# lblQubic/distributed_processor

Measured on AMD Instinct MI355X. Metric: emulated core-shots/s (config 2: 8-core Ramsey, 100 delays, 1e6 shots/GPU), higher is better.
Workload: dtype u32; 1 GPU; config2_ramsey_8core_100pt; shots_per_gpu=1000000, lane_order=shot-major, parallelism=shots sharded, 1 GPU(s)

## Files before the change

distributed_processor_amd/csrc/capi.cpp:

```cpp

#include <hip/hip_runtime.h>

#include <algorithm>
#include <cmath>
#include <cstdarg>
#include <cstdio>
#include <cstring>
#include <initializer_list>
#include <string>
#include <vector>

#include "kernels.h"
#include "launch_plan.h"
#include "lds_grants.h"
#include "program_image.h"

using namespace dpemu;

namespace dpemu {
static LdsGrants g_lds_grants;

hipError_t opt_in_dynamic_lds(const void *fn, size_t bytes)
{
    if (bytes <= LdsGrants::DEFAULT_LIMIT) return hipSuccess;
// ... 48 lines not shown
    uint32_t n_cu = 256;
    std::string err;
    uint4 *d_uops = nullptr;
    uint4 *d_uops_t = nullptr;
    uint4 *d_macro = nullptr;
    uint32_t *d_moff = nullptr;
    uint32_t *d_mchunk = nullptr, *d_mcoff = nullptr;
    uint32_t *d_offsets = nullptr, *d_ninstr = nullptr, *d_table = nullptr;
    ProgramFacts facts;
    uint32_t *d_ro_fq = nullptr;
    uint4 *d_ro_hdr = nullptr;
    uint32_t *d_thr = nullptr;
    uint64_t *d_lut = nullptr;
    std::vector<uint32_t> thr_cache;
    std::vector<uint64_t> lut_cache;
    int16_t *d_sin = nullptr;
    DevTable ch;
    DevTable dds_index;
    DevTable pairs;
    DevTable lines, fl_index;
    DevTable res;
    DevTable iqcols;
    uint32_t iq_wgs_per_cu = 0;
    DevTable trace_tab;
    uint32_t trace_wgs_per_cu = 0;
    DevTable qsim_tab;
    std::string last_kernel;
    bool timing = false;
    std::vector<std::pair<hipEvent_t, hipEvent_t>> ev_used, ev_free;
    DevTable hist_rep;
    bool hist_rep_dirty = true;
    hipEvent_t ord_ev = nullptr;
    hipStream_t ord_stream = nullptr;
    bool ord_valid = false;
};

static int fail(dpemu_ctx *ctx, int code, const char *fmt, ...)
{
    char buf[512];
    va_list ap;
    va_start(ap, fmt);
    vsnprintf(buf, sizeof buf, fmt, ap);
    va_end(ap);
    if (ctx) ctx->err = buf;
    return code;
}

#define HIPCHK(ctx, call)                                                                  \
    do {                                                                                   \
        hipError_t e_ = (call);                                                            \
        if (e_ != hipSuccess)                                                              \
            return fail(ctx, DPEMU_E_DEVICE, "%s: %s", #call, hipGetErrorString(e_));      \
    } while (0)

struct NamedPtr { const void *p; const char *name; };
static int check_ptrs(dpemu_ctx *ctx, const char *what, std::initializer_list<NamedPtr> ptrs)
{
    for (const NamedPtr &a : ptrs)
        if (a.name && !a.p) return fail(ctx, DPEMU_E_INVALID, "%s: %s is NULL", what, a.name);
    return DPEMU_OK;
}

static hipError_t order_begin(dpemu_ctx *ctx, hipStream_t s)
{
    if (ctx->ord_valid && s != ctx->ord_stream) return hipStreamWaitEvent(s, ctx->ord_ev, 0);
    return hipSuccess;
}

static hipError_t order_end(dpemu_ctx *ctx, hipStream_t s)
{
    const hipError_t e = hipEventRecord(ctx->ord_ev, s);
    ctx->ord_stream = s;
    ctx->ord_valid = e == hipSuccess;
    return e;
}

template <class Launch> static hipError_t timed(dpemu_ctx *ctx, hipStream_t stream, Launch launch)
{
    if (!ctx->timing) return launch();
    std::pair<hipEvent_t, hipEvent_t> e;
    if (!ctx->ev_free.empty()) {
        e = ctx->ev_free.back();
        ctx->ev_free.pop_back();
    } else {
        hipError_t r = hipEventCreate(&e.first);
        if (r != hipSuccess) return r;
        r = hipEventCreate(&e.second);
        if (r != hipSuccess) { (void)hipEventDestroy(e.first); return r; }
    }
    ctx->ev_used.push_back(e);
    hipError_t r = hipEventRecord(e.first, stream);
    if (r == hipSuccess) r = launch();
    if (r == hipSuccess) r = hipEventRecord(e.second, stream);
    return r;
}

template <class P> static void set_readout(P &p, const dpemu_config *cfg)
{
    p.seed = cfg->seed;
    p.meas_elem = cfg->meas_elem; p.ro_cpw = cfg->ro_cpw; p.ro_delay = cfg->ro_delay;
    p.ro_theta0 = cfg->ro_theta[0]; p.ro_theta1 = cfg->ro_theta[1];
    p.ro_gain0 = cfg->ro_gain[0]; p.ro_gain1 = cfg->ro_gain[1];
    p.ro_sigma = cfg->ro_sigma; p.ro_thr = cfg->ro_thr;
}

template <class T> static hipError_t to_device(T *&d, const uint32_t *src, uint64_t n)
{
// ... 31 lines not shown
    return DPEMU_OK;
}

int dpemu_create(int device, dpemu_ctx **out)
{
    if (!out) return DPEMU_E_INVALID;
    *out = nullptr;
    int n = 0;
    if (hipGetDeviceCount(&n) != hipSuccess || device < 0 || device >= n) return DPEMU_E_DEVICE;
    if (hipSetDevice(device) != hipSuccess) return DPEMU_E_DEVICE;
    dpemu_ctx *ctx = new dpemu_ctx();
    ctx->device = device;
    int cus = 0;
    if (hipDeviceGetAttribute(&cus, hipDeviceAttributeMultiprocessorCount, device) == hipSuccess && cus > 0)
        ctx->n_cu = (uint32_t)cus;
    std::vector<int16_t> lut(4096);
    dpemu_dds_sin_lut(lut.data());
    if (hipMalloc(&ctx->d_thr, 2 * DPEMU_MAX_CORES * sizeof(uint32_t)) != hipSuccess ||
        hipMalloc(&ctx->d_lut, 256 * sizeof(uint64_t)) != hipSuccess ||
        hipMalloc(&ctx->d_sin, 4096 * sizeof(int16_t)) != hipSuccess ||
        hipMemcpy(ctx->d_sin, lut.data(), 4096 * sizeof(int16_t), hipMemcpyHostToDevice) != hipSuccess ||
        hipEventCreateWithFlags(&ctx->ord_ev, hipEventDisableTiming) != hipSuccess) {
        dpemu_destroy(ctx);
        return DPEMU_E_NOMEM;
    }
    *out = ctx;
    return DPEMU_OK;
}

int dpemu_destroy(dpemu_ctx *ctx)
{
    if (!ctx) return DPEMU_E_INVALID;
    (void)hipSetDevice(ctx->device);
    if (ctx->ord_valid) (void)hipEventSynchronize(ctx->ord_ev);
    free_programs(ctx);
    (void)hipFree(ctx->d_thr); (void)hipFree(ctx->d_lut); (void)hipFree(ctx->d_sin);
    for (DevTable *t : {&ctx->ch, &ctx->dds_index, &ctx->pairs, &ctx->lines, &ctx->fl_index, &ctx->res, &ctx->iqcols,
                        &ctx->trace_tab, &ctx->qsim_tab, &ctx->hist_rep})
        t->release();
    for (auto *v : {&ctx->ev_used, &ctx->ev_free})
        for (auto &e : *v) { (void)hipEventDestroy(e.first); (void)hipEventDestroy(e.second); }
    if (ctx->ord_ev) (void)hipEventDestroy(ctx->ord_ev);
    delete ctx;
    return DPEMU_OK;
}

const char *dpemu_last_error(dpemu_ctx *ctx) { return ctx ? ctx->err.c_str() : "null context"; }

const char *dpemu_last_kernel(dpemu_ctx *ctx) { return ctx ? ctx->last_kernel.c_str() : ""; }

int dpemu_set_kernel_timing(dpemu_ctx *ctx, int enable)
{
    if (!ctx) return DPEMU_E_INVALID;
    ctx->timing = enable != 0;
    return DPEMU_OK;
}

int dpemu_kernel_times(dpemu_ctx *ctx, float *ms, int max_n, int *n_out)
{
    if (!ctx || (max_n > 0 && !ms)) return DPEMU_E_INVALID;
    HIPCHK(ctx, hipSetDevice(ctx->device));
    int n = 0;
    for (auto &e : ctx->ev_used) {
        HIPCHK(ctx, hipEventSynchronize(e.second));
        if (n < max_n) HIPCHK(ctx, hipEventElapsedTime(&ms[n], e.first, e.second));
        n++;
    }
    ctx->ev_free.insert(ctx->ev_free.end(), ctx->ev_used.begin(), ctx->ev_used.end());
    ctx->ev_used.clear();
    if (n_out) *n_out = n < max_n ? n : max_n;
    return DPEMU_OK;
}

int dpemu_load_programs(dpemu_ctx *ctx, const uint32_t *words, uint64_t n_cmds, const uint32_t *offsets,
                        const uint32_t *n_instr, uint32_t n_programs, const uint32_t *prog_table,
                        uint32_t n_groups, uint32_t cores_per_shot)
{
    if (!ctx) return DPEMU_E_INVALID;
    if ((!words && n_cmds) || !offsets || !n_instr || !prog_table || n_programs == 0 || n_groups == 0)
        return fail(ctx, DPEMU_E_INVALID, "load_programs: null array or empty program set");
    const uint32_t C = cores_per_shot;
    if (C == 0 || C > DPEMU_MAX_CORES || (C & (C - 1)))
        return fail(ctx, DPEMU_E_INVALID, "cores_per_shot %u is not a power of two in [1, 64]", C);
    if ((uint64_t)n_groups * C > 0xFFFFFFFFull) return fail(ctx, DPEMU_E_INVALID, "n_groups * C exceeds 2^32");
    for (uint32_t i = 0; i < n_programs; i++) {
        if (n_instr[i] > 65536u)
            return fail(ctx, DPEMU_E_INVALID, "program %u: %u commands exceed the 2^16-deep cmd_mem", i, n_instr[i]);
        if ((uint64_t)offsets[i] + n_instr[i] > n_cmds)
            return fail(ctx, DPEMU_E_INVALID, "program %u: offset %u + %u commands run past the %llu commands",
                        i, offsets[i], n_instr[i], (unsigned long long)n_cmds);
    }
    for (uint64_t i = 0; i < (uint64_t)n_groups * C; i++)
        if (prog_table[i] >= n_programs)
            return fail(ctx, DPEMU_E_INVALID, "prog_table[%llu] = %u >= n_programs", (unsigned long long)i, prog_table[i]);
    const ProgramImage im = build_program_image(words, offsets, n_instr, n_programs, prog_table, n_groups, C);
    if (!im.err.empty()) return fail(ctx, DPEMU_E_INVALID, "%s", im.err.c_str());
    HIPCHK(ctx, hipSetDevice(ctx->device));
    if (ctx->ord_valid) HIPCHK(ctx, hipEventSynchronize(ctx->ord_ev));
    free_programs(ctx);
    HIPCHK(ctx, to_device(ctx->d_uops, im.uops.data(), im.uops.size()));
    HIPCHK(ctx, to_device(ctx->d_uops_t, im.uops_t.data(), im.uops_t.size()));
    HIPCHK(ctx, to_device(ctx->d_macro, im.macro.data(), im.macro.size()));
    HIPCHK(ctx, to_device(ctx->d_moff, im.moff.data(), im.moff.size()));
    HIPCHK(ctx, to_device(ctx->d_mchunk, im.mchunk.data(), im.mchunk.size()));
    HIPCHK(ctx, to_device(ctx->d_mcoff, im.mcoff.data(), im.mcoff.size()));
    HIPCHK(ctx, to_device(ctx->d_offsets, im.goff.data(), n_programs));
    HIPCHK(ctx, to_device(ctx->d_ninstr, n_instr, n_programs));
    HIPCHK(ctx, to_device(ctx->d_table, prog_table, (uint64_t)n_groups * C));
    ctx->facts = im.facts;
    return DPEMU_OK;
}

int dpemu_load_readout_freqs(dpemu_ctx *ctx, const uint32_t *words, uint64_t n_words, const uint32_t *drv_off,
                             const uint32_t *drv_len, const uint32_t *lo_off, const uint32_t *lo_len)
{
    if (!ctx) return DPEMU_E_INVALID;
    if (!ctx->facts.n_programs) return fail(ctx, DPEMU_E_NOPROG, "load_readout_freqs before load_programs");
    if ((!words && n_words) || !drv_off || !drv_len || !lo_off || !lo_len)
        return fail(ctx, DPEMU_E_INVALID, "load_readout_freqs: null array");
    std::vector<uint32_t> hdr(4ull * ctx->facts.n_programs);
    for (uint32_t i = 0; i < ctx->facts.n_programs; i++) {
        if ((uint64_t)drv_off[i] + drv_len[i] > n_words || (uint64_t)lo_off[i] + lo_len[i] > n_words)
            return fail(ctx, DPEMU_E_INVALID, "load_readout_freqs: program %u's table runs past the %llu words", i,
                        (unsigned long long)n_words);
        hdr[4 * i] = drv_off[i]; hdr[4 * i + 1] = drv_len[i]; hdr[4 * i + 2] = lo_off[i]; hdr[4 * i + 3] = lo_len[i];
    }
    HIPCHK(ctx, hipSetDevice(ctx->device));
    if (ctx->ord_valid) HIPCHK(ctx, hipEventSynchronize(ctx->ord_ev));
    (void)hipFree(ctx->d_ro_fq);
    (void)hipFree(ctx->d_ro_hdr);
    ctx->d_ro_fq = nullptr;
    ctx->d_ro_hdr = nullptr;
    HIPCHK(ctx, hipMalloc(&ctx->d_ro_fq, std::max<uint64_t>(n_words, 1) * 4));
    if (n_words) HIPCHK(ctx, hipMemcpy(ctx->d_ro_fq, words, n_words * 4, hipMemcpyHostToDevice));
    HIPCHK(ctx, hipMalloc(&ctx->d_ro_hdr, hdr.size() * 4));
    HIPCHK(ctx, hipMemcpy(ctx->d_ro_hdr, hdr.data(), hdr.size() * 4, hipMemcpyHostToDevice));
    return DPEMU_OK;
}

static int validate(dpemu_ctx *ctx, const dpemu_config *cfg, uint64_t n_shots, bool want_hist)
{
    if (!cfg) return fail(ctx, DPEMU_E_INVALID, "null config");
    if (!ctx->facts.n_programs) return fail(ctx, DPEMU_E_NOPROG, "run before load_programs");
    if (cfg->cores_per_shot != ctx->facts.C)
        return fail(ctx, DPEMU_E_INVALID, "cores_per_shot %u != loaded %u", cfg->cores_per_shot, ctx->facts.C);
    if (cfg->n_groups != ctx->facts.n_groups)
        return fail(ctx, DPEMU_E_INVALID, "n_groups %u != loaded %u", cfg->n_groups, ctx->facts.n_groups);
    if (cfg->shots_per_group == 0) return fail(ctx, DPEMU_E_INVALID, "shots_per_group == 0");
    if (cfg->n_groups > 0x80000000u) return fail(ctx, DPEMU_E_INVALID, "n_groups > 2^31");
    if (cfg->max_cycles == 0 || cfg->max_cycles > 0x7FFFFFC0u)
        return fail(ctx, DPEMU_E_INVALID, "max_cycles must be in (0, 2^31 - 64]");
    if (cfg->meas_latency < 1 || cfg->meas_latency > (1u << 20) || cfg->sync_latency < 1 ||
        cfg->sync_latency > (1u << 20))
        return fail(ctx, DPEMU_E_INVALID, "meas_latency / sync_latency must be in [1, 2^20]");
    if (cfg->meas_model > DPEMU_MEAS_DEMOD)
        return fail(ctx, DPEMU_E_INVALID, "meas_model must be DPEMU_MEAS_STATE, _READOUT or _DEMOD");
    if (cfg->meas_model == DPEMU_MEAS_DEMOD) {
        if (cfg->ro_drv_elem > 3 || cfg->ro_drv_elem == cfg->meas_elem)
            return fail(ctx, DPEMU_E_INVALID, "ro_drv_elem %u must be an element 0..3 other than meas_elem",
                        cfg->ro_drv_elem);
        if (cfg->ro_cpw < 1 || cfg->ro_cpw > DPEMU_RO_CPW_MAX)
// ... 70 lines not shown
    p.n_shots = (uint32_t)n_shots;
    p.shot_major = cfg->lane_order == DPEMU_LANES_SHOT_MAJOR;
    p.C = C;
    p.log2C = 0;
    while ((1u << p.log2C) < C) p.log2C++;
    p.n_groups = cfg->n_groups; p.shots_per_group = cfg->shots_per_group;
    p.grp_g0 = (uint32_t)((shot_begin / cfg->shots_per_group) % cfg->n_groups);
    p.grp_r0 = (uint32_t)(shot_begin % cfg->shots_per_group);
    fast_div_init(cfg->shots_per_group, p.spg_div);
    fast_div_init(cfg->n_groups, p.ng_div);
    p.max_cycles = cfg->max_cycles;
    p.event_cap = cfg->event_cap;
    p.trace_cap = cfg->trace_cap;
    p.meas_cap = cfg->meas_cap;
    p.fproc_mode = cfg->fproc_mode;
    p.meas_latency = cfg->meas_latency; p.sync_latency = cfg->sync_latency;
    const uint64_t all = (C >= 64) ? ~0ull : ((1ull << C) - 1);
    p.sync_mask = cfg->sync_mask ? (cfg->sync_mask & all) : all;
    set_readout(p, cfg);
    p.meas_model = cfg->meas_model; p.ro_sep = cfg->ro_sep;
    p.ro_win = cfg->ro_win;
    p.ro_wrecip = cfg->ro_win ? (1u << 24) / cfg->ro_win : 0u;
    p.ro_drv_elem = cfg->ro_drv_elem;
    p.ro_axis = ctx->d_thr + DPEMU_MAX_CORES;
    p.ro_fq = ctx->d_ro_fq; p.ro_hdr = ctx->d_ro_hdr;
    p.acc = reinterpret_cast<int2 *>(out->acc);
    p.lut_mask = cfg->lut_mask;
    const uint64_t guard = (uint64_t)C * (cfg->max_cycles / 3u + 4u) + 1024u;
    p.iter_guard = guard > 0xFFFFFFF0ull ? 0xFFFFFFF0u : (uint32_t)guard;
    p.ev_stream = (cfg->exec_flags & DPEMU_X_STREAM_EVENTS) ? 1u : 0u;
    p.prog_lds_words = pl.prog_lds_words;
    if (pl.hist_repl) {
        const size_t cap0 = ctx->hist_rep.cap;
        HIPCHK(ctx, ctx->hist_rep.reserve((size_t)pl.R * pl.hist_stride * 4, stream));
        if (ctx->hist_rep.cap != cap0) ctx->hist_rep_dirty = true;
        if (ctx->hist_rep_dirty) {
            HIPCHK(ctx, hipMemsetAsync(ctx->hist_rep.d, 0, ctx->hist_rep.cap, stream));
            ctx->hist_rep_dirty = false;
        }
        p.hist = nullptr;
        p.hist_rep = ctx->hist_rep.as<uint32_t>();
        p.hist_reps = pl.R;
        p.hist_stride = pl.hist_stride;
        p.hist_lds = pl.hist_lds;
    }
    if (out->hist && !p.hist_rep && cfg->hist_assign)
        HIPCHK(ctx, hipMemsetAsync(out->hist, 0, pl.bins * sizeof(uint64_t), stream));
    if (p.hist_rep) ctx->hist_rep_dirty = true;
    HIPCHK(ctx, timed(ctx, stream, [&] {
        switch (pl.family) {
        case K_STRAIGHT: return launch_straight(p, pl.src, pl.fetch_batch, stream);
        case K_MACRO: return launch_macro(p, pl.slots, f.macro_nr, f.macro_addid, stream);
        case K_BRANCH: return launch_branch(p, pl.bfeat, stream);
        default: return launch_interp(p, pl.feat, stream);
        }
    }));
    ctx->last_kernel = pl.name;
    if (p.hist_rep) {
        HIPCHK(ctx, launch_hist_reduce(p.hist_rep, pl.R, pl.hist_stride, pl.bins, cfg->hist_assign != 0,
                                       reinterpret_cast<unsigned long long *>(out->hist), stream));
        ctx->hist_rep_dirty = false;
    }
    HIPCHK(ctx, order_end(ctx, stream));
    return DPEMU_OK;
}

int dpemu_run(dpemu_ctx *ctx, const dpemu_config *cfg, uint64_t shot_begin, uint64_t n_shots,
              const dpemu_outputs *out, void *stream)
{
    if (!ctx) return DPEMU_E_INVALID;
    if (!out) return fail(ctx, DPEMU_E_INVALID, "null outputs");
    int rc = validate(ctx, cfg, n_shots, out->hist != nullptr || out->hist_next != nullptr);
    if (rc) return rc;
    if (out->acc && cfg->meas_model != DPEMU_MEAS_DEMOD)
        return fail(ctx, DPEMU_E_INVALID, "acc: DEMOD runs only");
    if (out->hist_next) {
        const uint64_t bytes = ((uint64_t)cfg->n_groups << cfg->cores_per_shot) * sizeof(uint64_t);
        const uintptr_t a = (uintptr_t)out->hist, b = (uintptr_t)out->hist_next;
        if (out->hist && a < b + bytes && b < a + bytes)
            return fail(ctx, DPEMU_E_INVALID, "hist_next overlaps hist");
        if (b % sizeof(uint64_t)) return fail(ctx, DPEMU_E_INVALID, "hist_next is not 8-byte aligned");
    }
    if (n_shots == 0) {
        if (out->hist_next) {
            hipStream_t s = (hipStream_t)stream;
            HIPCHK(ctx, hipSetDevice(ctx->device));
            HIPCHK(ctx, order_begin(ctx, s));
            HIPCHK(ctx, hipMemsetAsync(out->hist_next, 0,
                                       ((size_t)cfg->n_groups << cfg->cores_per_shot) * sizeof(uint64_t), s));
            HIPCHK(ctx, order_end(ctx, s));
        }
        return DPEMU_OK;
    }
// ... 630 lines not shown
```

distributed_processor_amd/csrc/kernels.h:

```cpp
#pragma once

#include <hip/hip_runtime.h>
#include <stdint.h>

#include "../../include/dpemu.h"
#include "uop.h"

namespace dpemu {

constexpr uint32_t MEAS_LOOKUP = DPEMU_MEAS_LOOKUP;
constexpr uint32_t LUT_FIRE_CAP = DPEMU_LUT_FIRE_CAP;

__device__ __forceinline__ uint32_t block_exclusive_scan(uint32_t v, uint32_t *s_tmp, uint32_t *total)
{
    const uint32_t tid = threadIdx.x, wl = tid & 63, wv = tid >> 6;
    uint32_t x = v;
#pragma unroll
    for (int o = 1; o < 64; o <<= 1) {
        const uint32_t y = (uint32_t)__shfl_up((int)x, o, 64);
        if (wl >= (uint32_t)o) x += y;
    }
    if (wl == 63) s_tmp[wv] = x;
    __syncthreads();
    uint32_t off = 0, tot = 0;
// ... 28 lines not shown
    uint64_t reg_map;
    uint64_t reg_inv;
    uint32_t reg_used;
    uint32_t macro_rs;
    uint32_t macro_w3;
    const uint32_t *p1_thr;
    const uint64_t *lut_table;
    uint32_t *summary;
    uint4 *events;
    uint4 *trace;
    uint2 *meas;
    uint32_t *regs_out;
    unsigned long long *hist;
    uint64_t shot_begin;
    uint32_t n_lanes, n_shots, C, log2C, n_groups, shots_per_group;
    uint32_t shot_major;
    uint32_t grp_g0, grp_r0;
    uint32_t spg_div[3], ng_div[3];
    uint32_t max_cycles, event_cap, trace_cap, meas_cap;
    uint32_t fproc_mode, meas_elem, meas_latency, sync_latency;
    uint64_t sync_mask, seed;
    uint32_t lut_mask;
    uint32_t meas_model;
    int32_t ro_sep, ro_thr;
    uint32_t ro_sigma, ro_win, ro_wrecip;
    uint32_t ro_drv_elem, ro_cpw, ro_delay, ro_theta0, ro_theta1, ro_gain0, ro_gain1;
    const uint32_t *ro_axis;
    const uint32_t *ro_fq;
    const uint4 *ro_hdr;
    int2 *acc;
    uint32_t iter_guard;
    uint32_t ev_stream;
    uint32_t prog_lds_words;
    uint32_t *hist_rep;
    uint32_t hist_reps, hist_lds;
    uint64_t hist_stride;
    unsigned long long *hist_next;
    uint64_t hist_bins;
};

hipError_t launch_hist_reduce(uint32_t *rep, uint32_t R, uint64_t stride, uint64_t bins, bool assign,
                              unsigned long long *hist, hipStream_t stream);

hipError_t launch_interp(const KParams &p, int feat, hipStream_t stream);
hipError_t launch_straight(const KParams &p, int src, int fb, hipStream_t stream);
hipError_t opt_in_dynamic_lds(const void *fn, size_t bytes);
hipError_t launch_branch(const KParams &p, int feat, hipStream_t stream);
hipError_t launch_macro(const KParams &p, uint32_t slots, int nr, bool addid, hipStream_t stream);

struct DDSParams {
    const uint32_t *summary;
    const uint4 *events;
    const uint32_t *env, *freq;
    const int16_t *sin_lut;
    const uint32_t *ch;
    uint32_t *iq;
    uint32_t n_channels, n_lanes, n_samples, event_cap;
    uint32_t ev_lds;
    uint32_t rec_lds;
    uint32_t env_lds, freq_lds;
    uint32_t tiles;
    uint32_t stripes;
    uint32_t wg_tiles;
    uint4 *xs;
    uint32_t *xr;
    uint2 *cnt;
// ... 112 lines not shown
```

distributed_processor_amd/csrc/lane.h:

```cpp
#pragma once

#include "kernels.h"

namespace dpemu {

__device__ __forceinline__ uint4 sel4(bool c, uint4 a, uint4 b)
{
    return make_uint4(c ? a.x : b.x, c ? a.y : b.y, c ? a.z : b.z, c ? a.w : b.w);
}


#define INF32 0xFFFFFFFFu

__device__ __forceinline__ uint32_t bit_select(uint32_t m, uint32_t a, uint32_t b)
{
    return __builtin_amdgcn_bitop3_b32(m, a, b, 0xCA);
}

__device__ __forceinline__ void pulse_write(const uint4 u, uint32_t &pe, uint32_t &pp, uint32_t &pa)
{
    const int32_t w = (int32_t)u.w;
    const uint32_t m_env = (uint32_t)((w << 7) >> 31);
    const uint32_t m_cfg = (uint32_t)((w << 6) >> 31);
    const uint32_t m_ph = (uint32_t)((w << 5) >> 31);
// ... 262 lines not shown
        const uint32_t g = gx - fast_div(gx, p.ng_div) * p.n_groups;
        const uint32_t prog = p.prog_table[(uint64_t)g * C + (lo & (C - 1))];
        s_prog[idx] = p.uops[p.offsets[prog] + (idx - s_pref[lo])];
    }
    __syncthreads();
    const uint32_t sp = min(spos, spl);
    return s_pref[group_step(p, sp, sp0) * C + my_core];
}

__device__ __forceinline__ void block_core_major(const KParams &p, uint32_t &sl, uint32_t &core)
{
    const uint32_t S_log2 = 8u - p.log2C;
    if (p.shot_major) {
        core = threadIdx.x & (p.C - 1u);
        sl = (blockIdx.x << S_log2) + (threadIdx.x >> p.log2C);
    } else {
        core = threadIdx.x >> S_log2;
        sl = (blockIdx.x << S_log2) + (threadIdx.x & ((1u << S_log2) - 1u));
    }
}

__device__ __forceinline__ uint32_t shot_slot(const KParams &p)
{
    return p.shot_major ? threadIdx.x >> p.log2C : threadIdx.x & ((1u << (8u - p.log2C)) - 1u);
}

__device__ __forceinline__ void clear_hist_next(const KParams &p)
{
    if (!p.hist_next) return;
    const uint64_t n = (uint64_t)gridDim.x * BLOCK;
    for (uint64_t i = (uint64_t)blockIdx.x * BLOCK + threadIdx.x; i < p.hist_bins; i += n) p.hist_next[i] = 0ull;
}

__device__ __forceinline__ void count_outcome_block(const KParams &p, uint32_t *s_hist, uint32_t *s_key, bool valid,
                                                    uint32_t core, uint32_t sl, uint32_t grp, uint32_t last_bit)
{
    if (!p.hist && !p.hist_rep) return;
    const uint32_t tid = threadIdx.x, S_log2 = 8u - p.log2C, S = 1u << S_log2;
    const uint32_t slot = shot_slot(p);
    if (tid < S) s_key[tid] = 0u;
    __syncthreads();
    if (valid && last_bit) atomicOr(&s_key[slot], 1u << core);
    __syncthreads();
    const bool mine = valid && core == 0u;
    const uint32_t key = mine ? s_key[slot] : 0u;
    const uint64_t bin = (uint64_t)grp * (1ull << p.C) + key;
    if (p.hist_rep) {
        uint32_t *rep = p.hist_rep + (uint64_t)(blockIdx.x % p.hist_reps) * p.hist_stride;
        if (p.hist_lds) {
            if (mine) atomicAdd(&s_hist[bin], 1u);
            __syncthreads();
            const uint32_t bins = p.n_groups << p.C;
            for (uint32_t i = tid; i < bins; i += BLOCK)
                if (s_hist[i]) atomicAdd(&rep[i], s_hist[i]);
        } else if (mine) {
            atomicAdd(&rep[bin], 1u);
        }
    } else if (mine) {
        atomicAdd(&p.hist[bin], 1ull);
    }
    (void)sl;
}

__device__ __forceinline__ void write_summary(const KParams &p, uint32_t lane, uint32_t t_end, uint32_t ip,
                                              uint32_t status, uint32_t flags, uint32_t n_ev, uint32_t n_exec,
                                              uint32_t qclk_end, uint32_t n_meas, uint32_t meas_bits, uint32_t n_tr)
{
    uint4 *s = reinterpret_cast<uint4 *>(p.summary + 8ull * lane);
    const uint4 s0 = make_uint4(t_end, (ip & 0xFFFFu) | ((status & 0xFFu) << 16) | ((flags & 0xFFu) << 24), n_ev, n_exec);
    const uint4 s1 = make_uint4(qclk_end, n_meas, meas_bits, n_tr);
    s[0] = s0;
    s[1] = s1;
}

__device__ __forceinline__ void count_outcome(const KParams &p, uint32_t *s_hist, bool valid, uint32_t core,
                                              uint32_t grp, uint32_t last_bit)
{
    const uint32_t C = p.C, tid = threadIdx.x, wl = tid & 63;
    if (p.hist_rep) {
        const uint64_t key = group_bits(__ballot(last_bit != 0u), wl, C);
        const uint64_t bin = (uint64_t)grp * (1ull << C) + key;
        uint32_t *rep = p.hist_rep + (uint64_t)(blockIdx.x % p.hist_reps) * p.hist_stride;
        if (p.hist_lds) {
            if (valid && core == 0u) atomicAdd(&s_hist[bin], 1u);
            __syncthreads();
// ... 14 lines not shown
```

distributed_processor_amd/csrc/launch_plan.h:

```cpp
#pragma once

#include <algorithm>
#include <cmath>
#include <cstdio>
#include <cstring>
#include <string>
#include <vector>

#include "../../include/dpemu.h"
#include "program_image.h"

namespace dpemu {

enum KernelFamily { K_STRAIGHT, K_MACRO, K_BRANCH, K_INTERP };

struct RunPlan {
    KernelFamily family = K_INTERP;
    bool cmd_major = false;
    int src = STRAIGHT_PROG, fetch_batch = 1;
    uint32_t slots = 0;
    int feat = 0, bfeat = 0;
    uint32_t prog_lds_words = 0;
    bool hist_repl = false;
    uint32_t R = 0;
    uint64_t bins = 0, hist_stride = 0;
    uint32_t hist_lds = 0;
    std::string name;
};

inline RunPlan plan_run(const ProgramFacts &f, const dpemu_config *cfg, uint64_t n_shots, bool want_hist)
{
    RunPlan pl;
    const uint32_t C = cfg->cores_per_shot;
    const uint32_t n_lanes = (uint32_t)(n_shots * C);
    const bool cmd_major = pl.cmd_major = f.has_cmd_major && !(cfg->exec_flags & DPEMU_X_PROG_MAJOR);
    const uint32_t S = BLOCK / C, ng = cfg->n_groups;
    const uint64_t w = (ng == 1) ? 1 : (S - 1) / cfg->shots_per_group + 2;
    uint64_t footprint = ~0ull;
    if (w * C <= BLOCK) {
        const std::vector<uint64_t> &gl = f.group_len;
        uint64_t tot = 0;
        for (uint64_t x : gl) tot += x;
        footprint = (w / ng) * tot;
        const uint64_t r = w % ng;
        if (r) {
            uint64_t win = 0, best = 0;
            for (uint64_t i = 0; i < r; i++) win += gl[i % ng];
            best = win;
            for (uint64_t g = 1; g < ng; g++) {
                win += gl[(g + r - 1) % ng];
                win -= gl[g - 1];
                best = std::max(best, win);
            }
            footprint += best;
        }
    }
    int feat = 0;
    const uint64_t blocks = ((uint64_t)n_lanes + BLOCK - 1) / BLOCK;
    const bool small = blocks <= 4 * 256;
    pl.fetch_batch = small ? 4 : 1;
// ... 26 lines not shown
    } else if (footprint <= PROG_LDS_MAX && (cfg->exec_flags & DPEMU_X_PROG_LDS)) {
        feat |= FEAT_PROG_LDS;
        pl.prog_lds_words = (uint32_t)std::max<uint64_t>(16, (footprint + 15) & ~15ull);
    }
    if (f.has_fproc) feat |= (cfg->fproc_mode == DPEMU_FPROC_LUT) ? FEAT_LUT : FEAT_FPROC;
    if (f.has_sync) feat |= FEAT_SYNC;
    if (f.straight) feat |= FEAT_STRAIGHT;
    pl.feat = feat;
    if (want_hist) {
        pl.bins = (uint64_t)ng << C;
        const uint64_t spg = std::max<uint64_t>(1, cfg->shots_per_group);
        const uint64_t live_groups = std::min<uint64_t>(ng, (65536 / C) / spg + 1);
        bool repl = (live_groups << C) < 4096;
        if (cfg->exec_flags & DPEMU_X_HIST_DIRECT) repl = false;
        if (cfg->exec_flags & DPEMU_X_HIST_REPL) repl = true;
        if (repl) {
            const uint64_t stride = (pl.bins + 31) & ~31ull;
            pl.hist_repl = true;
            pl.R = (uint32_t)std::min<uint64_t>({64, blocks, std::max<uint64_t>(1, (2ull << 20) / (stride * 4))});
            pl.hist_stride = stride;
            pl.hist_lds = pl.bins <= HIST_LDS_MAX && (BLOCK / C) >= 4 * pl.bins;
        }
    }
    const bool branch = !uniform && !macro && !(cfg->exec_flags & (DPEMU_X_GENERAL | DPEMU_X_PROG_LDS));
    pl.bfeat = (feat & (FEAT_FPROC | FEAT_LUT | FEAT_SYNC)) | (f.reg_writes ? FEAT_REGS : 0) | (demod ? FEAT_DEMOD : 0);
    if (branch) {
        pl.prog_lds_words = 0;
        if (footprint <= BRANCH_LDS_MAX && !(cfg->exec_flags & DPEMU_X_PROG_MAJOR)) {
            pl.bfeat |= FEAT_PROG_LDS;
            pl.prog_lds_words = (uint32_t)std::max<uint64_t>(16, (footprint + 15) & ~15ull);
        }
    }
    pl.family = uniform ? K_STRAIGHT : macro ? K_MACRO : branch ? K_BRANCH : K_INTERP;
    char name[96];
    if (uniform)
        snprintf(name, sizeof name, "straight_kernel<%s,fb%d>",
                 pl.src == STRAIGHT_ROWS ? "rows" : pl.src == STRAIGHT_PROG ? "prog" : "lds", pl.fetch_batch);
    else if (macro && pl.slots)
        snprintf(name, sizeof name, "macro_staged_kernel<%d%s%s>", f.macro_nr, f.macro_addid ? ",addid" : "",
                 pl.slots > MACRO_SLOTS ? ",12" : "");
    else if (macro)
        snprintf(name, sizeof name, "macro_kernel");
    else if (branch)
        snprintf(name, sizeof name, "branch_kernel<feat=0x%x%s>", pl.bfeat, C == 8 ? ",c8" : "");
    else
        snprintf(name, sizeof name, "interp_kernel<feat=0x%x>", feat);
    pl.name = name;
    return pl;
}

struct DdsPlan {
    uint32_t ev_lds, rec_lds, env_lds, freq_lds, tiles, stripes, wg_tiles;
    bool dense;
};

inline DdsPlan plan_dds(const uint32_t *desc, uint32_t n_channels, uint32_t n_samples, uint32_t event_cap)
{
    uint32_t env_max = 0, freq_max = 0;
    for (uint32_t i = 0; i < n_channels; i++) {
        const uint32_t *d = desc + (size_t)i * DDS_CH_WORDS;
        const uint32_t ew = d[3] == 1 ? dds_env_pairs_words(d[5]) : d[5], fw = 2 * d[7];
        if (ew <= DDS_ENV_LDS_MAX) env_max = std::max(env_max, ew);
        if (fw <= DDS_FREQ_LDS_MAX) freq_max = std::max(freq_max, fw);
    }
    DdsPlan p{};
    p.ev_lds = std::max<uint32_t>(8, (event_cap + 7) & ~7u);
// ... 165 lines not shown
```

distributed_processor_amd/csrc/straight.hip:

```cpp

#include <hip/hip_runtime.h>
#include <stdint.h>

#include "lane.h"

namespace dpemu {


template <int SRC, int FB>
__global__ void __launch_bounds__(BLOCK) straight_kernel(const KParams p)
{
    constexpr bool ROWS = SRC == STRAIGHT_ROWS, LDS = SRC == STRAIGHT_LDS;
    __shared__ uint32_t s_hist[HIST_LDS_MAX];
    __shared__ uint32_t s_pref[LDS ? BLOCK + 1 : 1];
    __shared__ uint32_t s_scan[BLOCK / 64];
    __shared__ uint32_t s_key[BLOCK];
    extern __shared__ uint4 s_prog[];
    const uint32_t tid = threadIdx.x;
    const uint32_t C = p.C;
    uint32_t sl, core;
    clear_hist_next(p);
    block_core_major(p, sl, core);
    const bool valid = sl < p.n_shots;
    const uint32_t lane = out_lane(p, sl, core);
    const uint64_t shot = p.shot_begin + sl;
    const uint32_t n_lanes = p.n_lanes;

    uint32_t grp = 0, prog = 0, base = 0, nprog = 0;
    if (valid) {
        grp = shot_group(p, sl);
        prog = p.prog_table[(uint64_t)grp * C + core];
        nprog = p.n_instr[prog];
        if (!ROWS) base = p.offsets[prog];
    }
    const uint32_t thr = valid ? p.p1_thr[core] : 0u;
    if (p.hist_lds) {
        for (uint32_t i = tid; i < HIST_LDS_MAX; i += BLOCK) s_hist[i] = 0;
        __syncthreads();
    }
    if constexpr (LDS) base = stage_programs(p, s_prog, s_pref, s_scan, sl, core);

    const uint32_t max_cycles = p.max_cycles;
// ... 101 lines not shown
        case 0xB:
            emit(live, t, 1u);
            t = live ? t + 3u : t;
            break;
        case 0x0: case 0xA:
            st = live ? ST_DONE : st;
            k_end = live ? k : k_end;
            break;
        default:
            retire(u, k, false, live);
        }
    };

    retire(fetch(0u), 0u, true, st == 0u);
    for (uint32_t k = 1; __ballot(st == 0u); k += FB) {
        uint4 u[FB];
#pragma unroll
        for (int j = 0; j < FB; j++) u[j] = fetch(k + j);
#pragma unroll
        for (int j = 0; j < FB; j++) {
            if (j && !__ballot(st == 0u)) break;
            step(u[j], k + j);
        }
    }
    flags |= (n_ev > p.event_cap ? F_EVENT_OVF : 0u) | (n_meas > min(p.meas_cap, MEAS_LOOKUP) ? F_MEAS_OVF : 0u);

    if (valid && p.summary)
        write_summary(p, lane, t, k_end, st & 0xFFu, flags, n_ev, k_end + ((st & ST_TOP) ? 0u : 1u),
                      t < 1u ? 0u : t - 1u, n_meas, meas_bits, 0u);
    if (valid && p.regs_out) {
#pragma unroll
        for (int r = 0; r < 16; r++) p.regs_out[(uint64_t)r * n_lanes + lane] = 0u;
    }
    count_outcome_block(p, s_hist, s_key, valid, core, sl, grp, last_bit);
}

template <int SRC, int FB>
static hipError_t launch_src(const KParams &p, uint32_t blocks, size_t shmem, hipStream_t stream)
{
    const hipError_t e = opt_in_dynamic_lds((const void *)straight_kernel<SRC, FB>, shmem);
    if (e != hipSuccess) return e;
    hipLaunchKernelGGL((straight_kernel<SRC, FB>), dim3(blocks), dim3(BLOCK), shmem, stream, p);
    return hipGetLastError();
}

hipError_t launch_straight(const KParams &p, int src, int fb, hipStream_t stream)
{
    const uint32_t blocks = (uint32_t)((p.n_lanes + BLOCK - 1) / BLOCK);
    if (blocks == 0) return hipSuccess;
    const size_t shmem = src == STRAIGHT_LDS ? (size_t)p.prog_lds_words * sizeof(uint4) : 0;
#define SRC_CASE(S)                                                                                    \
    case S: return fb == 1 ? launch_src<S, 1>(p, blocks, shmem, stream) : launch_src<S, 4>(p, blocks, shmem, stream);
    switch (src) {
    SRC_CASE(STRAIGHT_ROWS) SRC_CASE(STRAIGHT_PROG) SRC_CASE(STRAIGHT_LDS)
    }
#undef SRC_CASE
    return hipErrorInvalidValue;
}

}
```

distributed_processor_amd/csrc/uop.h:

```cpp
#pragma once

#include <stdint.h>

#if defined(__HIPCC__)
#define DPEMU_HD __host__ __device__
#else
#define DPEMU_HD
#endif

namespace dpemu {

constexpr uint32_t BLOCK = 256;

constexpr int FEAT_FPROC = 1;
constexpr int FEAT_SYNC = 2;
constexpr int FEAT_LUT = 4;
constexpr int FEAT_PROG_LDS = 8;
constexpr int FEAT_STRAIGHT = 16;
constexpr int FEAT_REGS = 32;
constexpr int FEAT_DEMOD = 64;
constexpr uint32_t PROG_LDS_MAX = 1024;
constexpr uint32_t BRANCH_LDS_MAX = 512;

constexpr uint32_t UOP_RS_ENV = 1u << 16, UOP_RS_PH = 1u << 17, UOP_RS_FR = 1u << 18, UOP_RS_AMP = 1u << 19;
// ... 5 lines not shown
    const uint32_t rs0 = (w[3] >> 20) & 15u;
    u[0] = (op4 == 0x9 || op4 == 0xC) ? ((w[0] >> 5) | (w[1] << 27)) : ((w[2] >> 24) | (w[3] << 8));
    u[1] = (op4 << 28) | ((w[3] >> 24) & 7u) | (((w[3] >> 27) & 1u) << 3) | (((w[2] >> 20) & 15u) << 4) |
           (((w[2] >> 16) & 15u) << 8);
    u[2] = ((w[2] >> 4) & 0xFFFFu) | (((w[1] >> 20) & 0xFFu) << 16);
    u[3] = rs0 << 20;
    if (op4 == 0x8 || op4 == 0x9) {
        const uint32_t env_i = ((w[2] >> 26) | (w[3] << 6)) & 0xFFFFFFu, ph_i = (w[2] >> 7) & 0x1FFFFu;
        const uint32_t fr_i = ((w[1] >> 28) | (w[2] << 4)) & 0x1FFu, amp_i = (w[1] >> 10) & 0xFFFFu;
        const uint32_t cfg_i = (w[1] >> 5) & 0xFu;
        const uint32_t env_we = (w[3] >> 19) & 1u, env_rs = (w[3] >> 18) & 1u;
        const uint32_t ph_we = (w[2] >> 25) & 1u, ph_rs = (w[2] >> 24) & 1u;
        const uint32_t fr_we = (w[2] >> 6) & 1u, fr_rs = (w[2] >> 5) & 1u;
        const uint32_t amp_we = (w[1] >> 27) & 1u, amp_rs = (w[1] >> 26) & 1u;
        const uint32_t cfg_we = (w[1] >> 9) & 1u;
        const uint32_t rs = (env_we & env_rs) | ((ph_we & ph_rs) << 1) | ((fr_we & fr_rs) << 2) | ((amp_we & amp_rs) << 3);
        u[1] = (op4 << 28) | (env_we && !env_rs ? env_i : 0u) | (cfg_we ? cfg_i << 24 : 0u);
        u[2] = (ph_we && !ph_rs ? ph_i : 0u) | (fr_we && !fr_rs ? fr_i << 17 : 0u);
        u[3] = (rs0 << 20) | (amp_we && !amp_rs ? amp_i : 0u) | (rs << 16) | (env_we << 24) | (cfg_we << 25) |
               (ph_we << 26) | (fr_we << 27) | (amp_we << 28) | ((rs ? 1u : 0u) << 29);
    }
}

inline void fast_div_init(uint32_t d, uint32_t out[3])
{
    uint32_t l = 0;
    while (l < 32 && (1ull << l) < d) l++;
    out[0] = (uint32_t)(((1ull << 32) * ((1ull << l) - d)) / d + 1);
    out[1] = l < 1 ? l : 1u;
    out[2] = l > 1 ? l - 1 : 0u;
}

constexpr uint32_t HIST_LDS_MAX = 1024;

enum { STRAIGHT_ROWS = 0, STRAIGHT_PROG = 1, STRAIGHT_LDS = 2 };
constexpr uint32_t STRAIGHT_LDS_MAX = 9216;

constexpr uint32_t MACRO_SLOTS = 8;
constexpr uint32_t MACRO_SLOTS_WIDE = 12;
constexpr uint32_t MACRO_CHUNK = 16;
constexpr uint32_t MACRO_ABSENT = 0x80000000u;
constexpr uint32_t MACRO_SIMPLE = 0x40000000u;
constexpr uint32_t MACRO_CHUNK_MIXED = 0xFFFFFFFFu;
constexpr uint32_t W3_OP = 0, W3_IN0 = 3, W3_RS1 = 4, W3_RD = 5, W3_RS0 = 6, W3_INC = 7, W3_PRES = 8;
DPEMU_HD inline uint32_t w3_ctl(uint32_t packed, int k)
{
    const uint32_t f = packed >> (10 * k);
    return (f & 0x1Fu) | (((f >> W3_RD) & 1u) << 8) | (((f >> W3_RS0) & 1u) << 12) | (((f >> W3_INC) & 1u) << 30) |
           (((f >> W3_PRES) & 1u) << 31);
}
DPEMU_HD inline uint32_t w3_pack(uint32_t ctl)
{
    if (!(ctl >> 31)) return 0u;
    return (ctl & 0x1Fu) | (((ctl >> 8) & 1u) << W3_RD) | (((ctl >> 12) & 1u) << W3_RS0) |
           (((ctl >> 30) & 1u) << W3_INC) | (1u << W3_PRES);
}

constexpr uint32_t DDS_CH_WORDS = 8;
constexpr uint32_t DDS_MAX_EVENTS = 1024;
constexpr uint32_t DDS_TILE = 4 * BLOCK;
#ifndef DDS_TILES_PER_STRIPE
#define DDS_TILES_PER_STRIPE 16u
#endif
constexpr uint32_t DDS_ENV_LDS_MAX = 8192;
constexpr uint32_t DDS_FREQ_LDS_MAX = 2048;

// ... 61 lines not shown
```

Before: 55.42 billion core-shots/s.

## Fold replicated histogram reduction into straight kernel via last-block ticket

For uniform programs using replicated LDS histograms, the straight kernel now folds replicas itself. Each block adds its counts to a replica row, and ticket counters pick the final block, which reduces all replicas into the output histogram. This removes the separate hist_reduce launch. Ordering-event recording is also deferred on the null stream, cutting per-call event records. In exchange the tail block does serialized reduction work, and correctness depends on the ticket and relaxed-atomic scheme.

```diff
diff --git a/distributed_processor_amd/csrc/capi.cpp b/distributed_processor_amd/csrc/capi.cpp
--- a/distributed_processor_amd/csrc/capi.cpp
+++ b/distributed_processor_amd/csrc/capi.cpp
@@ -104,7 +104,7 @@
     bool hist_rep_dirty = true;
     hipEvent_t ord_ev = nullptr;
     hipStream_t ord_stream = nullptr;
-    bool ord_valid = false;
+    bool ord_valid = false, ord_pending = false;
 };
 
 static int fail(dpemu_ctx *ctx, int code, const char *fmt, ...)
@@ -133,18 +133,35 @@
     return DPEMU_OK;
 }
 
-static hipError_t order_begin(dpemu_ctx *ctx, hipStream_t s)
-{
-    if (ctx->ord_valid && s != ctx->ord_stream) return hipStreamWaitEvent(s, ctx->ord_ev, 0);
-    return hipSuccess;
-}
-
-static hipError_t order_end(dpemu_ctx *ctx, hipStream_t s)
-{
-    const hipError_t e = hipEventRecord(ctx->ord_ev, s);
-    ctx->ord_stream = s;
+static hipError_t order_mark(dpemu_ctx *ctx)
+{
+    if (!ctx->ord_pending) return hipSuccess;
+    const hipError_t e = hipEventRecord(ctx->ord_ev, ctx->ord_stream);
+    ctx->ord_pending = false;
     ctx->ord_valid = e == hipSuccess;
     return e;
+}
+
+static hipError_t order_begin(dpemu_ctx *ctx, hipStream_t s)
+{
+    if (s == ctx->ord_stream) return hipSuccess;
+    const hipError_t e = order_mark(ctx);
+    if (e != hipSuccess) return e;
+    return ctx->ord_valid ? hipStreamWaitEvent(s, ctx->ord_ev, 0) : hipSuccess;
+}
+
+static hipError_t order_end(dpemu_ctx *ctx, hipStream_t s)
+{
+    ctx->ord_stream = s;
+    ctx->ord_pending = true;
+    return s ? order_mark(ctx) : hipSuccess;
+}
+
+static hipError_t order_sync(dpemu_ctx *ctx)
+{
+    const hipError_t e = order_mark(ctx);
+    if (e != hipSuccess) return e;
+    return ctx->ord_valid ? hipEventSynchronize(ctx->ord_ev) : hipSuccess;
 }
 
 template <class Launch> static hipError_t timed(dpemu_ctx *ctx, hipStream_t stream, Launch launch)
@@ -242,7 +259,7 @@
 {
     if (!ctx) return DPEMU_E_INVALID;
     (void)hipSetDevice(ctx->device);
-    if (ctx->ord_valid) (void)hipEventSynchronize(ctx->ord_ev);
+    (void)order_sync(ctx);
     free_programs(ctx);
     (void)hipFree(ctx->d_thr); (void)hipFree(ctx->d_lut); (void)hipFree(ctx->d_sin);
     for (DevTable *t : {&ctx->ch, &ctx->dds_index, &ctx->pairs, &ctx->lines, &ctx->fl_index, &ctx->res, &ctx->iqcols,
@@ -306,7 +323,7 @@
     const ProgramImage im = build_program_image(words, offsets, n_instr, n_programs, prog_table, n_groups, C);
     if (!im.err.empty()) return fail(ctx, DPEMU_E_INVALID, "%s", im.err.c_str());
     HIPCHK(ctx, hipSetDevice(ctx->device));
-    if (ctx->ord_valid) HIPCHK(ctx, hipEventSynchronize(ctx->ord_ev));
+    HIPCHK(ctx, order_sync(ctx));
     free_programs(ctx);
     HIPCHK(ctx, to_device(ctx->d_uops, im.uops.data(), im.uops.size()));
     HIPCHK(ctx, to_device(ctx->d_uops_t, im.uops_t.data(), im.uops_t.size()));
@@ -336,7 +353,7 @@
         hdr[4 * i] = drv_off[i]; hdr[4 * i + 1] = drv_len[i]; hdr[4 * i + 2] = lo_off[i]; hdr[4 * i + 3] = lo_len[i];
     }
     HIPCHK(ctx, hipSetDevice(ctx->device));
-    if (ctx->ord_valid) HIPCHK(ctx, hipEventSynchronize(ctx->ord_ev));
+    HIPCHK(ctx, order_sync(ctx));
     (void)hipFree(ctx->d_ro_fq);
     (void)hipFree(ctx->d_ro_hdr);
     ctx->d_ro_fq = nullptr;
@@ -473,13 +490,14 @@
     p.prog_lds_words = pl.prog_lds_words;
     if (pl.hist_repl) {
         const size_t cap0 = ctx->hist_rep.cap;
-        HIPCHK(ctx, ctx->hist_rep.reserve((size_t)pl.R * pl.hist_stride * 4, stream));
+        HIPCHK(ctx, ctx->hist_rep.reserve((size_t)pl.hist_rep_words() * 4, stream));
         if (ctx->hist_rep.cap != cap0) ctx->hist_rep_dirty = true;
         if (ctx->hist_rep_dirty) {
             HIPCHK(ctx, hipMemsetAsync(ctx->hist_rep.d, 0, ctx->hist_rep.cap, stream));
             ctx->hist_rep_dirty = false;
         }
-        p.hist = nullptr;
+        if (!pl.hist_fold) p.hist = nullptr;
+        p.hist_fold = !pl.hist_fold ? 0u : cfg->hist_assign ? HIST_FOLD_ASSIGN : HIST_FOLD_ADD;
         p.hist_rep = ctx->hist_rep.as<uint32_t>();
         p.hist_reps = pl.R;
         p.hist_stride = pl.hist_stride;
@@ -498,8 +516,9 @@
     }));
     ctx->last_kernel = pl.name;
     if (p.hist_rep) {
-        HIPCHK(ctx, launch_hist_reduce(p.hist_rep, pl.R, pl.hist_stride, pl.bins, cfg->hist_assign != 0,
-                                       reinterpret_cast<unsigned long long *>(out->hist), stream));
+        if (!pl.hist_fold)
+            HIPCHK(ctx, launch_hist_reduce(p.hist_rep, pl.R, pl.hist_stride, pl.bins, cfg->hist_assign != 0,
+                                           reinterpret_cast<unsigned long long *>(out->hist), stream));
         ctx->hist_rep_dirty = false;
     }
     HIPCHK(ctx, order_end(ctx, stream));
diff --git a/distributed_processor_amd/csrc/kernels.h b/distributed_processor_amd/csrc/kernels.h
--- a/distributed_processor_amd/csrc/kernels.h
+++ b/distributed_processor_amd/csrc/kernels.h
@@ -84,6 +84,7 @@
     uint32_t iter_guard;
     uint32_t ev_stream;
     uint32_t prog_lds_words;
+    uint32_t hist_fold;
     uint32_t *hist_rep;
     uint32_t hist_reps, hist_lds;
     uint64_t hist_stride;
diff --git a/distributed_processor_amd/csrc/lane.h b/distributed_processor_amd/csrc/lane.h
--- a/distributed_processor_amd/csrc/lane.h
+++ b/distributed_processor_amd/csrc/lane.h
@@ -318,6 +318,47 @@
     for (uint64_t i = (uint64_t)blockIdx.x * BLOCK + threadIdx.x; i < p.hist_bins; i += n) p.hist_next[i] = 0ull;
 }
 
+__device__ __forceinline__ void fold_replicas(const KParams &p, uint32_t *s_hist, uint32_t bins)
+{
+    constexpr int RLX = __ATOMIC_RELAXED, AGENT = __HIP_MEMORY_SCOPE_AGENT;
+    const uint32_t wl = threadIdx.x, R = p.hist_reps, row = blockIdx.x % R;
+    uint32_t *rep = p.hist_rep + (uint64_t)row * p.hist_stride;
+    for (uint32_t i = wl; i < bins; i += 64)
+        if (s_hist[i]) __hip_atomic_fetch_add(&rep[i], s_hist[i], RLX, AGENT);
+    asm volatile("s_waitcnt vmcnt(0)" ::: "memory");
+    uint32_t *ticket = p.hist_rep + (uint64_t)R * p.hist_stride;
+    const uint32_t n_row = (gridDim.x - row + R - 1u) / R;
+    uint32_t last = 0;
+    if (wl == 0) {
+        uint32_t *t = ticket + row * HIST_TICKET_PITCH, *tr = ticket + R * HIST_TICKET_PITCH;
+        if (__hip_atomic_fetch_add(t, 1u, RLX, AGENT) == n_row - 1u) {
+            __hip_atomic_exchange(t, 0u, RLX, AGENT);
+            if (__hip_atomic_fetch_add(tr, 1u, RLX, AGENT) == R - 1u) {
+                __hip_atomic_exchange(tr, 0u, RLX, AGENT);
+                last = 1;
+            }
+        }
+    }
+    if (!__builtin_amdgcn_readfirstlane(last)) return;
+    for (uint32_t i = wl; i < bins; i += 64) s_hist[i] = 0;
+    __builtin_amdgcn_wave_barrier();
+    for (uint32_t x0 = wl; x0 - wl < bins * R; x0 += 64 * 8) {
+        uint32_t v[8], b[8];
+#pragma unroll
+        for (int k = 0; k < 8; k++) {
+            const uint32_t x = x0 + 64u * k, r = x / bins;
+            b[k] = x - r * bins;
+            v[k] = x < bins * R ? __hip_atomic_exchange(&p.hist_rep[(uint64_t)r * p.hist_stride + b[k]], 0u, RLX, AGENT) : 0u;
+        }
+#pragma unroll
+        for (int k = 0; k < 8; k++)
+            if (v[k]) atomicAdd(&s_hist[b[k]], v[k]);
+    }
+    __builtin_amdgcn_wave_barrier();
+    for (uint32_t i = wl; i < bins; i += 64) p.hist[i] = (p.hist_fold == HIST_FOLD_ASSIGN ? 0ull : p.hist[i]) + s_hist[i];
+}
+
+template <bool FOLD = false>
 __device__ __forceinline__ void count_outcome_block(const KParams &p, uint32_t *s_hist, uint32_t *s_key, bool valid,
                                                     uint32_t core, uint32_t sl, uint32_t grp, uint32_t last_bit)
 {
@@ -337,6 +378,12 @@
             if (mine) atomicAdd(&s_hist[bin], 1u);
             __syncthreads();
             const uint32_t bins = p.n_groups << p.C;
+            if constexpr (FOLD) {
+                if (p.hist_fold) {
+                    if (tid < 64u) fold_replicas(p, s_hist, bins);
+                    return;
+                }
+            }
             for (uint32_t i = tid; i < bins; i += BLOCK)
                 if (s_hist[i]) atomicAdd(&rep[i], s_hist[i]);
         } else if (mine) {
diff --git a/distributed_processor_amd/csrc/launch_plan.h b/distributed_processor_amd/csrc/launch_plan.h
--- a/distributed_processor_amd/csrc/launch_plan.h
+++ b/distributed_processor_amd/csrc/launch_plan.h
@@ -25,7 +25,10 @@
     uint32_t R = 0;
     uint64_t bins = 0, hist_stride = 0;
     uint32_t hist_lds = 0;
+    bool hist_fold = false;
     std::string name;
+
+    uint64_t hist_rep_words() const { return R * hist_stride + (hist_fold ? (R + 1ull) * HIST_TICKET_PITCH : 0); }
 };
 
 inline RunPlan plan_run(const ProgramFacts &f, const dpemu_config *cfg, uint64_t n_shots, bool want_hist)
@@ -118,6 +121,7 @@
         }
     }
     pl.family = uniform ? K_STRAIGHT : macro ? K_MACRO : branch ? K_BRANCH : K_INTERP;
+    pl.hist_fold = uniform && pl.hist_repl && pl.hist_lds;
     char name[96];
     if (uniform)
         snprintf(name, sizeof name, "straight_kernel<%s,fb%d>",
diff --git a/distributed_processor_amd/csrc/straight.hip b/distributed_processor_amd/csrc/straight.hip
--- a/distributed_processor_amd/csrc/straight.hip
+++ b/distributed_processor_amd/csrc/straight.hip
@@ -7,7 +7,7 @@
 namespace dpemu {
 
 
-template <int SRC, int FB>
+template <int SRC, int FB, bool FOLD>
 __global__ void __launch_bounds__(BLOCK) straight_kernel(const KParams p)
 {
     constexpr bool ROWS = SRC == STRAIGHT_ROWS, LDS = SRC == STRAIGHT_LDS;
@@ -175,15 +175,15 @@
 #pragma unroll
         for (int r = 0; r < 16; r++) p.regs_out[(uint64_t)r * n_lanes + lane] = 0u;
     }
-    count_outcome_block(p, s_hist, s_key, valid, core, sl, grp, last_bit);
-}
-
-template <int SRC, int FB>
+    count_outcome_block<FOLD>(p, s_hist, s_key, valid, core, sl, grp, last_bit);
+}
+
+template <int SRC, int FB, bool FOLD>
 static hipError_t launch_src(const KParams &p, uint32_t blocks, size_t shmem, hipStream_t stream)
 {
-    const hipError_t e = opt_in_dynamic_lds((const void *)straight_kernel<SRC, FB>, shmem);
+    const hipError_t e = opt_in_dynamic_lds((const void *)straight_kernel<SRC, FB, FOLD>, shmem);
     if (e != hipSuccess) return e;
-    hipLaunchKernelGGL((straight_kernel<SRC, FB>), dim3(blocks), dim3(BLOCK), shmem, stream, p);
+    hipLaunchKernelGGL((straight_kernel<SRC, FB, FOLD>), dim3(blocks), dim3(BLOCK), shmem, stream, p);
     return hipGetLastError();
 }
 
@@ -193,7 +193,10 @@
     if (blocks == 0) return hipSuccess;
     const size_t shmem = src == STRAIGHT_LDS ? (size_t)p.prog_lds_words * sizeof(uint4) : 0;
 #define SRC_CASE(S)                                                                                    \
-    case S: return fb == 1 ? launch_src<S, 1>(p, blocks, shmem, stream) : launch_src<S, 4>(p, blocks, shmem, stream);
+    case S:                                                                                            \
+        if (p.hist_fold)                                                                               \
+            return fb == 1 ? launch_src<S, 1, true>(p, blocks, shmem, stream) : launch_src<S, 4, true>(p, blocks, shmem, stream); \
+        return fb == 1 ? launch_src<S, 1, false>(p, blocks, shmem, stream) : launch_src<S, 4, false>(p, blocks, shmem, stream);
     switch (src) {
     SRC_CASE(STRAIGHT_ROWS) SRC_CASE(STRAIGHT_PROG) SRC_CASE(STRAIGHT_LDS)
     }
diff --git a/distributed_processor_amd/csrc/uop.h b/distributed_processor_amd/csrc/uop.h
--- a/distributed_processor_amd/csrc/uop.h
+++ b/distributed_processor_amd/csrc/uop.h
@@ -61,6 +61,8 @@
 }
 
 constexpr uint32_t HIST_LDS_MAX = 1024;
+constexpr uint32_t HIST_TICKET_PITCH = 32;
+enum { HIST_FOLD_ADD = 1, HIST_FOLD_ASSIGN = 2 };
 
 enum { STRAIGHT_ROWS = 0, STRAIGHT_PROG = 1, STRAIGHT_LDS = 2 };
 constexpr uint32_t STRAIGHT_LDS_MAX = 9216;
```

After: 56.38 billion core-shots/s (median of 6 runs). 1.02x the previous value.
